# envoy/ksql

Hardware: AMD Instinct MI355X
Metric: records/sec, windowed GROUP BY (COUNT(*) TUMBLING 5 s GROUP BY card_number HAVING > 3) (higher is better)
Workload: dtype int64

## Files before the change

### ksql_amd/csrc/khip_agg_c1.hip

```cpp
#include <algorithm>
#include <cstdio>
#include <type_traits>
#include <vector>

#include "khip_part.hpp"

namespace khip {

constexpr int C1_TILE = 65536;
constexpr int C1_NT = 512;
constexpr int C1_CH = 8192;
template <class T>
__device__ __forceinline__ T c1_ld(const T* p) {
  return *p;
}
constexpr int C1_SEGMAX = 512;
constexpr int C1_SEGB = 7;
constexpr int C1_SEGOF = 512;
constexpr uint32_t C1_SENT = 0x80000000u;

__device__ __forceinline__ int bits_of(uint64_t v) { return v ? 64 - __clzll((long long)v) : 0; }

__device__ __forceinline__ int64_t ci_ld(const int64_t* ci, int k) {
  const uint64_t v = (uint64_t)__hip_atomic_load(&ci[k], __ATOMIC_RELAXED, __HIP_MEMORY_SCOPE_AGENT);
// ... 761 lines not shown
      for (int u = 0; u < AU; u++) any |= (uint32_t)sb[u] <= li[u];
      if (!__ballot(any)) break;
      for (int u = 0; u < AU; u++) {
        const bool on = (uint32_t)sb[u] <= li[u];
        lo[u] += on ? 1 : 0;
        ba[u] = on ? (uint32_t)(sb[u] >> 32) : ba[u];
        sb[u] = sg2[lo[u] + 1];
      }
    }
#pragma unroll
    for (int u = 0; u < AU; u++) at[u] = ba[u] + li[u];
  } else {
    uint32_t lo[AU], hi[AU];
#pragma unroll
    for (int u = 0; u < AU; u++) {
      lo[u] = 0u;
      hi[u] = (uint32_t)nseg;
    }
    for (int span = nseg; span > 1; span = (span + 1) >> 1) {
      uint32_t pm[AU];
#pragma unroll
      for (int u = 0; u < AU; u++) pm[u] = (uint32_t)sg2[(lo[u] + hi[u]) >> 1];
#pragma unroll
      for (int u = 0; u < AU; u++) {
        const uint32_t mid = (lo[u] + hi[u]) >> 1;
        const bool up = pm[u] <= li[u];
        lo[u] = up ? mid : lo[u];
        hi[u] = up ? hi[u] : mid;
      }
    }
#pragma unroll
    for (int u = 0; u < AU; u++) at[u] = (uint32_t)(sg2[lo[u]] >> 32) + li[u];
  }
}

template <int NT, int AU, class ID, bool WIDE>
__global__ __launch_bounds__(NT, 4) void k_c1_merge(
    C1Q q, const uint32_t* __restrict__ work, int64_t nwork, const int64_t* __restrict__ bb,
    const int* __restrict__ cstart, const uint16_t* __restrict__ seg, const uint64_t* __restrict__ srec, int first,
    uint64_t* __restrict__ buf0, uint64_t* __restrict__ buf1, const uint8_t* __restrict__ sel,
    const int64_t* __restrict__ cnt, unsigned long long* __restrict__ newcnt, uint8_t* __restrict__ fail,
    unsigned long long* __restrict__ need, int64_t close0, uint64_t* __restrict__ closed,
    unsigned long long* __restrict__ closed_n, unsigned long long closed_cap, const int64_t* __restrict__ ci,
    unsigned long long* __restrict__ hnew,
    unsigned long long* __restrict__ hclosed, uint32_t* __restrict__ prn, const uint32_t* __restrict__ srecT,
    unsigned long long* __restrict__ dbg) {
  if (ci_ld(ci, CI_GATE) == 0) return;
  if ((ci_ld(ci, CI_WIDE) != 0) != WIDE) return;
  if (!WIDE && (ci_ld(ci, CI_ID32) != 0) != (sizeof(ID) == 4)) return;
  static_assert(!WIDE || sizeof(ID) == 8, "wide records use 64-bit identities");
  constexpr int NW = NT / 64;
  constexpr ID EMPTY = (ID)~(ID)0;
  const int log2H = q.log2H;
  const int H = 1 << log2H;
  const int lane = threadIdx.x & 63, wave = threadIdx.x >> 6;
  extern __shared__ __attribute__((aligned(16))) char smem[];
  KLDS ID* ids = (KLDS ID*)(KLDS char*)smem;
  KLDS uint32_t* rt = (KLDS uint32_t*)((KLDS char*)smem + (size_t)(H + 64) * sizeof(ID));
  KLDS uint32_t* ct = rt + (H + 64);
  KLDS uint16_t* list = (KLDS uint16_t*)(ct + (H + 64));
  KLDS uint64_t* sg2 = (KLDS uint64_t*)((KLDS char*)list + (((size_t)H * 2 + 15) & ~(size_t)15));
  KLDS int64_t* lbb = (KLDS int64_t*)(sg2 + C1_SEGMAX + 4);
  KLDS int32_t* lcs = (KLDS int32_t*)(lbb + (1 << (q.log2P - q.fbits)) + 1);
  KLDS uint16_t* segof = (KLDS uint16_t*)(lcs + (1 << (q.log2P - q.fbits)) + 2);
  __shared__ int lovf, nnew;
  __shared__ int wsum[NW], csum[NW];
  __shared__ unsigned long long lbase, cbase;
  const int F = 1 << q.fbits;
  const int64_t wbase = ci_ld(ci, CI_WBASE), whi = ci_ld(ci, CI_WHI), T0 = ci_ld(ci, CI_T0), tmin = ci_ld(ci, CI_TMIN);
  const int wbits = (int)ci_ld(ci, CI_WBITS);
  const int64_t kmin = ci_ld(ci, CI_KMINC);
  const uint64_t krange = (uint64_t)ci_ld(ci, CI_KRANGE);
  const int32_t tmin32 = (int32_t)(tmin - T0);
  const int64_t wstart = wbase * q.adv;
  const bool r32 = ci_ld(ci, CI_TMAX) - wstart < ((int64_t)1 << 32);
  const uint32_t tsh32 = (uint32_t)(T0 - wstart);
  const bool evict = close0 != INT64_MIN;
  C1M_T0;
  const uint32_t dummy = (uint32_t)H + (uint32_t)lane;
  for (int i = threadIdx.x; i < H + 64; i += NT) {
    ids[i] = EMPTY;
    rt[i] = 0u;
    ct[i] = 0u;
  }
  if (threadIdx.x == 0) {
    lovf = 0;
    nnew = 0;
  }
  auto row_id = [&](const uint64_t* row, ID* id, uint32_t* h) -> bool {
    const int64_t wi = (int64_t)fast_udiv((uint64_t)row[1], q.fd) - wbase;
    if constexpr (WIDE) {
      if (wi < 0 || wi > whi) {
        *h = (uint32_t)(key_hash((int64_t)row[0]) >> 32) ^ (uint32_t)row[1];
        return false;
      }
      *id = (ID)((key_hash((int64_t)row[0]) << q.log2P) | (uint64_t)wi);
      *h = c1_hash<ID>(*id);
      return true;
    }
    const uint64_t krel = (uint64_t)((int64_t)row[0] - kmin);
    if (krel > krange || wi < 0 || wi > whi) {
      *h = (uint32_t)(key_hash((int64_t)row[0]) >> 32) ^ (uint32_t)row[1];
      return false;
    }
    if constexpr (sizeof(ID) == 4) *id = (ID)(((uint32_t)krel << wbits) | (uint32_t)wi);
    else *id = (ID)((krel << 32) | (uint64_t)wi);
    *h = c1_hash<ID>(*id);
    return true;
  };
  struct Pre {
    uint32_t p;
    int sbits, sub;
    int64_t nrow;
    uint32_t selw;
    uint32_t s0, s1;
  };
  auto bucket = [&](uint32_t p, int& cs, int64_t& bb0) -> int {
    const int b = (int)(p >> q.fbits);
    cs = lcs[b];
    bb0 = lbb[b];
    const int nseg = lcs[b + 1] - cs;
    return nseg < 0 || nseg > C1_SEGMAX ? 0 : nseg;
  };
  struct It {
    uint32_t p;
    int sbits, sub, nseg, segb;
    uint32_t rn;
    uint32_t bb0;
    int64_t nrow;
    bool isel;
  };
  auto fetch = [&](int64_t w, Pre& r) {
    uint32_t p;
    int sbits = 0, sub = 0;
    if (work) {
      const uint32_t x = work[w];
      p = x & 0xFFFFu;
      sbits = (x >> 16) & 0xF;
      sub = (int)(x >> 20);
    } else {
      p = (uint32_t)w;
    }
    p = __builtin_amdgcn_readfirstlane(p);
    const int f = (int)(p & (uint32_t)(F - 1));
    int cs;
    int64_t bb0;
    const int nseg = bucket(p, cs, bb0);
    r.p = p;
    r.sbits = sbits;
    r.sub = sub;
    r.nrow = cnt[p];
    r.selw = ((const uint32_t*)sel)[p >> 2];
    const int k0 = threadIdx.x * 2;
    r.s0 = r.s1 = 0u;
    if (k0 < nseg) {
      const uint16_t* sg = seg + (int64_t)(cs + k0) * (F + 1) + f;
      r.s0 = (uint32_t)sg[0] | (uint32_t)sg[1] << 16;
    }
    if (k0 + 1 < nseg) {
      const uint16_t* sg = seg + (int64_t)(cs + k0 + 1) * (F + 1) + f;
      r.s1 = (uint32_t)sg[0] | (uint32_t)sg[1] << 16;
    }
  };
  auto prep = [&](const Pre& r, It& it) {
    int cs;
    int64_t bb0;
    const int nseg = bucket(r.p, cs, bb0);
    it.p = r.p;
    it.sbits = r.sbits;
    it.sub = r.sub;
    it.nrow = r.nrow;
    it.isel = ((r.selw >> (8 * (r.p & 3))) & 0xFFu) != 0;
    const int k0 = threadIdx.x * 2;
    const uint32_t s00 = r.s0 & 0xFFFFu, s10 = r.s1 & 0xFFFFu;
    const int len0 = k0 < nseg ? (int)(r.s0 >> 16) - (int)s00 : 0;
    const int len1 = k0 + 1 < nseg ? (int)(r.s1 >> 16) - (int)s10 : 0;
    const uint32_t base0 = (uint32_t)(k0 * C1_CH) + s00;
    const uint32_t base1 = (uint32_t)((k0 + 1) * C1_CH) + s10;
    const int s = len0 + len1;
    int incl = s;
    for (int off = 1; off < 64; off <<= 1) {
      const int y = __shfl_up(incl, off, 64);
      if (lane >= off) incl += y;
    }
    if (lane == 63) wsum[wave] = incl;
    lds_barrier();
    int before = 0;
    int tot = 0;
    for (int k = 0; k < NW; k++) {
      before += k < wave ? wsum[k] : 0;
      tot += wsum[k];
    }
    const int ex = before + incl - s;
    const int segb = tot <= (C1_SEGOF << 5) ? 5 : (tot <= (C1_SEGOF << 6) ? 6 : C1_SEGB);
    const int bm = (1 << segb) - 1;
    if (k0 < nseg) sg2[k0] = (uint32_t)ex | (uint64_t)(base0 - (uint32_t)ex) << 32;
    if (k0 + 1 < nseg) sg2[k0 + 1] = (uint32_t)(ex + len0) | (uint64_t)(base1 - (uint32_t)(ex + len0)) << 32;
    for (int bj = (ex + bm) >> segb, be = (ex + len0 + bm) >> segb; bj < be && bj < C1_SEGOF; bj++)
      segof[bj] = (uint16_t)k0;
    for (int bj = (ex + len0 + bm) >> segb, be = (ex + s + bm) >> segb; bj < be && bj < C1_SEGOF; bj++)
      segof[bj] = (uint16_t)(k0 + 1);
    if (k0 < nseg && k0 + 2 >= nseg) sg2[nseg] = (uint32_t)(ex + s);
    if (nseg == 0 && threadIdx.x == 0) sg2[0] = 0u;
    lds_barrier();
    it.rn = __builtin_amdgcn_readfirstlane((uint32_t)sg2[nseg]);
    it.segb = __builtin_amdgcn_readfirstlane(segb);
    it.nseg = __builtin_amdgcn_readfirstlane(nseg);
    it.bb0 = __builtin_amdgcn_readfirstlane((uint32_t)bb0);
  };
  uint64_t ra[AU], rb[AU];
  uint32_t ta[AU], tb[AU];
  auto load = [&](uint64_t (&x)[AU], uint32_t (&tx)[AU], uint32_t l0, const It& t) {
    uint32_t at[AU];
    c1_seg_lookup<AU, NT>(sg2, segof, l0, t.rn, t.nseg, t.segb, at);
    const char* sb = (const char*)(srec + t.bb0);
#pragma unroll
    for (int u = 0; u < AU; u++) x[u] = c1_ld((const uint64_t*)(sb + (uint64_t)(uint32_t)(at[u] << 3)));
    if constexpr (WIDE) {
      const char* sbT = (const char*)(srecT + t.bb0);
#pragma unroll
      for (int u = 0; u < AU; u++) tx[u] = c1_ld((const uint32_t*)(sbT + (uint64_t)(uint32_t)(at[u] << 2)));
    }
  };
  auto load01 = [&](const It& x) {
    if (x.rn > 0) load(ra, ta, 0u, x);
    if (x.rn > (uint32_t)(AU * NT)) load(rb, tb, (uint32_t)(AU * NT), x);
  };
  for (int k = threadIdx.x; k <= (1 << (q.log2P - q.fbits)); k += NT) {
    lcs[k] = cstart[k];
    lbb[k] = bb[k];
  }
  lds_barrier();
  Pre pr{};
  It nx{};
  if (blockIdx.x < nwork) {
    fetch(blockIdx.x, pr);
    prep(pr, nx);
    load01(nx);
  }
  for (int64_t w = blockIdx.x; w < nwork; w += gridDim.x) {
    const It it = nx;
    const uint32_t p = it.p;
    const int sbits = it.sbits, sub = it.sub;
    const uint32_t rn = it.rn;
    const int64_t nrow = it.nrow;
    const bool isel = it.isel;
    const int64_t wn = w + gridDim.x;
    if (wn < nwork) fetch(wn, pr);
    if (first && threadIdx.x == 0) prn[p] = rn;
    if (rn == 0 && first) {
      if (wn < nwork) {
        prep(pr, nx);
        load01(nx);
      }
      continue;
    }
    const uint64_t* src = (isel ? buf1 : buf0) + (uint64_t)p * q.cmax * q.sw;
    auto evict_failed = [&]() {
      if (!first || !evict || nrow == 0) return;
      auto mine_closed = [&](const uint64_t* row) -> bool {
        if ((int64_t)row[1] + q.size > close0) return false;
        if (!sbits) return true;
        ID id;
        uint32_t h;
        row_id(row, &id, &h);
        return (int)c1_sub(h, sbits) == sub;
      };
      int n_cl = 0;
      for (int64_t r = threadIdx.x; r < nrow; r += NT) n_cl += mine_closed(src + r * q.sw) ? 1 : 0;
      const int wave_cl = (int)wave_sum(n_cl);
      if (lane == 0) csum[wave] = wave_cl;
      lds_barrier();
      int cl_before = 0, cl_total = 0;
      for (int k = 0; k < NW; k++) {
        if (k < wave) cl_before += csum[k];
        cl_total += csum[k];
      }
      if (threadIdx.x == 0)
        cbase = c1_reserve_closed(closed_n, (unsigned long long)cl_total, closed_cap, &fail[p], need);
      lds_barrier();
      const unsigned long long cb = cbase;
      if (cl_total == 0 || cb == C1_NOSLOT) return;
      uint64_t ccur = cb + (uint64_t)cl_before;
      const uint64_t lt = (1ULL << lane) - 1;
      int nhc = 0;
      for (int64_t r0 = wave * 64; r0 < nrow; r0 += NT) {
        const int64_t r = r0 + lane;
        const uint64_t* row = src + (r < nrow ? r : 0) * q.sw;
        const bool cl = r < nrow && mine_closed(row);
        const uint64_t bc = __ballot(cl);
        if (cl) {
          uint64_t* cd = closed + (ccur + __popcll(bc & lt)) * q.sw;
          for (int k = 0; k < q.sw; k++) cd[k] = row[k];
          nhc += q.hv_active && c1q_having(q, row[3]) ? 1 : 0;
        }
        ccur += __popcll(bc);
      }
      if (q.hv_active) {
        nhc = (int)wave_sum(nhc);
        if (lane == 0 && nhc) atomicAdd(hclosed, (unsigned long long)nhc);
      }
    };
    C1M_T(0);
    auto apply = [&](const uint64_t (&xr)[AU], const uint32_t (&txr)[AU], uint32_t l0, auto R32, auto&& prefetch) -> bool {
      ID id[AU];
      uint32_t e[AU], tr[AU];
      bool pend[AU], claimed[AU];
#pragma unroll
      for (int u = 0; u < AU; u++) {
        const uint32_t li = l0 + threadIdx.x + (uint32_t)(u * NT);
        const uint64_t v = xr[u];
        const int32_t t32 = WIDE ? (int32_t)txr[u] : (int32_t)(uint32_t)v;
        const uint64_t krel = v >> 32;
        uint64_t wi;
        if constexpr (decltype(R32)::value) wi = fast_udiv32((uint32_t)t32 + tsh32, q.fd32);
        else wi = fast_udiv((uint64_t)(T0 + (int64_t)t32), q.fd) - (uint64_t)wbase;
        ID x;
        if constexpr (WIDE) x = (ID)((v << q.log2P) | wi);
        else if constexpr (sizeof(ID) == 4) x = (ID)(((uint32_t)krel << wbits) | (uint32_t)wi);
        else x = (ID)((krel << 32) | wi);
        const uint32_t h = c1_hash<ID>(x);
        bool act = li < rn;
        if (sbits) act = act && (int)c1_sub(h, sbits) == sub;
        id[u] = act ? x : EMPTY;
        e[u] = act ? h >> (32 - log2H) : dummy;
        tr[u] = (uint32_t)(t32 - tmin32) + 1u;
      }
      ID old[AU];
#pragma unroll
      for (int u = 0; u < AU; u++) {
        old[u] = EMPTY;
        __hip_atomic_compare_exchange_strong(&ids[e[u]], &old[u], id[u], __ATOMIC_RELAXED, __ATOMIC_RELAXED,
                                             __HIP_MEMORY_SCOPE_WORKGROUP);
      }
      const int fullv = *(volatile KLDS int*)&lovf;
      prefetch();
      const int full = __builtin_amdgcn_readfirstlane(fullv);
#pragma unroll
      for (int u = 0; u < AU; u++) {
        claimed[u] = id[u] != EMPTY && old[u] == EMPTY;
        pend[u] = old[u] != EMPTY && old[u] != id[u];
      }
      for (int probes = 1;; probes++) {
        bool anyp = false;
#pragma unroll
        for (int u = 0; u < AU; u++) anyp |= pend[u];
        if (!__ballot(anyp)) break;
        if (probes >= H) {
          lovf = 1;
#pragma unroll
          for (int u = 0; u < AU; u++)
            if (pend[u]) id[u] = EMPTY;
          break;
        }
#pragma unroll
        for (int u = 0; u < AU; u++) {
          if (!pend[u]) continue;
          e[u] = (e[u] + 1) & (uint32_t)(H - 1);
          ID o2 = EMPTY;
          __hip_atomic_compare_exchange_strong(&ids[e[u]], &o2, id[u], __ATOMIC_RELAXED, __ATOMIC_RELAXED,
                                               __HIP_MEMORY_SCOPE_WORKGROUP);
          claimed[u] = o2 == EMPTY;
          pend[u] = o2 != EMPTY && o2 != id[u];
        }
      }
      int nnow;
      {
        bool cl[AU];
#pragma unroll
        for (int u = 0; u < AU; u++) cl[u] = claimed[u] && id[u] != EMPTY;
        nnow = mg_list_append_n<AU>(cl, e, list, &nnew);
      }
#pragma unroll
      for (int u = 0; u < AU; u++) {
        if (id[u] == EMPTY) continue;
        __hip_atomic_fetch_max(&rt[e[u]], tr[u], WG_RLX);
        __hip_atomic_fetch_add(&ct[e[u]], 1u, WG_RLX);
      }
      return !full && nnow <= q.hmax;
    };
    constexpr uint32_t CR = (uint32_t)(AU * NT);
    const uint32_t nch = (rn + CR - 1u) / CR;
    if (rn > 0) {
      for (uint32_t c = 0; c < nch; c += 2) {
        auto pa = [&] { if (c + 2 < nch) load(ra, ta, (c + 2) * CR, it); };
        const bool ga = r32 ? apply(ra, ta, c * CR, std::true_type{}, pa) : apply(ra, ta, c * CR, std::false_type{}, pa);
        if (!ga || c + 1 >= nch) break;
        auto pb = [&] { if (c + 3 < nch) load(rb, tb, (c + 3) * CR, it); };
        const bool gb = r32 ? apply(rb, tb, (c + 1) * CR, std::true_type{}, pb)
                            : apply(rb, tb, (c + 1) * CR, std::false_type{}, pb);
        if (!gb) break;
      }
    }
    lds_barrier();
    if (wn < nwork) {
      prep(pr, nx);
      load01(nx);
    }
    C1M_T(1);
    const int nl = nnew < H ? nnew : H;
    if (lovf || nnew > q.hmax) {
      if (threadIdx.x == 0) fail[p] |= 1;
      for (int i = threadIdx.x; i < nl; i += NT) {
        const uint32_t e = list[i];
        ids[e] = EMPTY;
        rt[e] = 0u;
        ct[e] = 0u;
      }
      evict_failed();
      lds_barrier();
      if (threadIdx.x == 0) {
        lovf = 0;
        nnew = 0;
      }
      lds_barrier();
      continue;
    }
    int n_mine = 0, n_cl = 0;
    for (int64_t r = threadIdx.x; r < nrow; r += NT) {
      const uint64_t* row = src + r * q.sw;
      ID id;
      uint32_t h;
      const bool has = row_id(row, &id, &h);
      if (sbits && (int)c1_sub(h, sbits) != sub) continue;
      if (evict && (int64_t)row[1] + q.size <= close0) {
        n_cl += first ? 1 : 0;
        continue;
      }
      if (has) {
        const int e = c1_find_id<ID>(ids, id, h >> (32 - log2H), H);
        if (e >= 0) rt[e] |= RT_MATCHED;
      }
      n_mine++;
    }
    if (nrow > 0) lds_barrier();
    const int per = ((nl + NW - 1) / NW + 63) & ~63;
    const int lb0 = wave * per, lb1 = lb0 + per < nl ? lb0 + per : nl;
    int nnw = 0;
    for (int k = lb0; k < lb1; k += 64) {
      const int i = k + lane;
      const uint32_t e = i < lb1 ? list[i] : dummy;
      const bool isnew = i < lb1 && !(rt[e] & RT_MATCHED);
      nnw += (int)__popcll(__ballot(isnew));
    }
    const int wave_rows = (int)wave_sum(n_mine) + nnw;
    const int wave_cl = (int)wave_sum(n_cl);
    if (lane == 0) {
      wsum[wave] = wave_rows;
      csum[wave] = wave_cl;
    }
    lds_barrier();
    int wave_before = 0, total = 0, cl_before = 0, cl_total = 0;
    for (int k = 0; k < NW; k++) {
      if (k < wave) wave_before += wsum[k], cl_before += csum[k];
      total += wsum[k];
      cl_total += csum[k];
    }
    if (threadIdx.x == 0) {
      if (work) lbase = total ? atomicAdd(&newcnt[p], (unsigned long long)total) : 0ULL;
      else {
        lbase = 0;
        newcnt[p] = (unsigned long long)total;
      }
      cbase = (int64_t)(lbase + total) <= q.cmax
                  ? c1_reserve_closed(closed_n, (unsigned long long)cl_total, closed_cap, &fail[p], need)
                  : 0ULL;
    }
    lds_barrier();
    if ((int64_t)(lbase + total) > q.cmax) {
      if (threadIdx.x == 0) {
        fail[p] |= 2;
        atomicMax(need, (unsigned long long)(lbase + total));
      }
      for (int i = threadIdx.x; i < nl; i += NT) {
        const uint32_t e = list[i];
        ids[e] = EMPTY;
        rt[e] = 0u;
        ct[e] = 0u;
      }
      evict_failed();
      lds_barrier();
      if (threadIdx.x == 0) nnew = 0;
      lds_barrier();
      continue;
    }
    C1M_T(3);
    uint64_t* dst0 = (isel ? buf0 : buf1) + (uint64_t)p * q.cmax * q.sw;
    uint64_t cur = lbase + (uint64_t)wave_before;
    uint64_t ccur = cbase + (uint64_t)cl_before;
    const bool cmove = first && cbase != C1_NOSLOT;
    const uint64_t lt = (1ULL << lane) - 1;
    int nh = 0, nhc = 0;
    for (int64_t r0 = wave * 64; r0 < nrow; r0 += NT) {
      const int64_t r = r0 + lane;
      const uint64_t* row = src + (r < nrow ? r : 0) * q.sw;
      bool live = r < nrow, cl = false;
      int e = -1;
      if (live) {
        ID id;
        uint32_t h;
        const bool has = row_id(row, &id, &h);
        if (sbits) live = (int)c1_sub(h, sbits) == sub;
        cl = live && evict && (int64_t)row[1] + q.size <= close0;
        live = live && !cl;
        if (live && has) e = c1_find_id<ID>(ids, id, h >> (32 - log2H), H);
      }
      const uint64_t bc = __ballot(cl);
      if (cl && cmove) {
        uint64_t* cd = closed + (ccur + __popcll(bc & lt)) * q.sw;
        for (int k = 0; k < q.sw; k++) cd[k] = row[k];
        nhc += q.hv_active && c1q_having(q, row[3]) ? 1 : 0;
      }
      ccur += __popcll(bc);
      const uint64_t bl = __ballot(live);
      if (live) {
        const uint64_t ri = cur + __popcll(bl & lt);
        uint64_t* dst = dst0 + ri * q.sw;
        uint64_t w2 = row[2], c = row[3];
        if (e >= 0) {
          const int64_t t = tmin + (int64_t)(rt[e] & ~RT_MATCHED) - 1;
          w2 = t > (int64_t)w2 ? (uint64_t)t : w2;
          c += ct[e];
        }
        *(longlong2*)dst = make_longlong2((int64_t)row[0], (int64_t)row[1]);
        *(longlong2*)(dst + 2) = make_longlong2((int64_t)w2, (int64_t)c);
        const bool now = !q.hv_active || c1q_having(q, c);
        nh += q.hv_active && now ? 1 : 0;
        if (q.chg)
          q.chg[(uint64_t)p * q.cmax + ri] =
              e >= 0 ? (uint8_t)(CHG_TOUCHED | (!q.hv_active || c1q_having(q, row[3]) ? CHG_OLD : 0) | (now ? CHG_NEW : 0))
                     : (uint8_t)0;
      }
      cur += __popcll(bl);
    }
    if (nrow > 0) lds_barrier();
    const uint32_t wmask = wbits ? (1u << wbits) - 1u : 0u;
    for (int k = lb0; k < lb1; k += 64) {
      const int i = k + lane;
      const uint32_t e = i < lb1 ? list[i] : dummy;
      const uint32_t rv = rt[e];
      const bool used = i < lb1;
      const bool isnew = used && !(rv & RT_MATCHED);
      const uint64_t bl = __ballot(isnew);
      if (isnew) {
        const uint64_t ri = cur + __popcll(bl & lt);
        uint64_t* dst = dst0 + ri * q.sw;
        const ID id = ids[e];
        int64_t key, wi;
        if constexpr (WIDE) {
          wi = (int64_t)((uint64_t)id & (((uint64_t)1 << q.log2P) - 1));
          key = key_of_hash(((uint64_t)p << (64 - q.log2P)) | ((uint64_t)id >> q.log2P));
        } else if constexpr (sizeof(ID) == 4) {
          key = kmin + (int64_t)((uint32_t)id >> wbits);
          wi = (int64_t)((uint32_t)id & wmask);
        } else {
          key = kmin + (int64_t)((uint64_t)id >> 32);
          wi = (int64_t)((uint64_t)id & 0xFFFFFFFFull);
        }
        const uint32_t c = ct[e];
        *(longlong2*)dst = make_longlong2(key, (wbase + wi) * q.adv);
        *(longlong2*)(dst + 2) = make_longlong2(tmin + (int64_t)rv - 1, (int64_t)c);
        const bool now = !q.hv_active || c1q_having(q, c);
        nh += q.hv_active && now ? 1 : 0;
        if (q.chg) q.chg[(uint64_t)p * q.cmax + ri] = (uint8_t)(CHG_TOUCHED | (now ? CHG_NEW : 0));
      }
      if (used) {
        ids[e] = EMPTY;
        rt[e] = 0u;
        ct[e] = 0u;
      }
      cur += __popcll(bl);
    }
    if (q.hv_active) {
      nh = (int)wave_sum(nh);
      nhc = (int)wave_sum(nhc);
      if (lane == 0 && nh) atomicAdd(&hnew[p], (unsigned long long)nh);
      if (lane == 0 && nhc) atomicAdd(hclosed, (unsigned long long)nhc);
    }
    lds_barrier();
    C1M_T(4);
    if (threadIdx.x == 0) nnew = 0;
    lds_barrier();
  }
}

constexpr int C1V_CH = 4096;
constexpr int C1V_MAXW = 8;

typedef uint64_t c1v_u2 __attribute__((ext_vector_type(2)));
__device__ __forceinline__ ulonglong2 ld_nt2(const ulonglong2* p) {
  const c1v_u2 v = c1_ld((const c1v_u2*)p);
  return make_ulonglong2(v.x, v.y);
}

struct C1VCol {
  const void* data;
  const uint8_t* valid;
  int32_t type;
};


template <int U, int NT, bool ST, bool ROWS>
__global__ __launch_bounds__(NT) __attribute__((amdgpu_waves_per_eu(4))) void k_c1v_scatter(
    const int64_t* __restrict__ keys, const int64_t* __restrict__ ts, const uint8_t* __restrict__ kv,
    const uint8_t* __restrict__ rv, C1VCol vc, RowsIn ri, int64_t n, int64_t nT, int log2B, uint16_t* __restrict__ rloc,
    uint16_t* __restrict__ roff, uint32_t* __restrict__ ttot, ulonglong2* __restrict__ srec, int64_t* __restrict__ tilestat,
    int64_t* __restrict__ tpart, int64_t* __restrict__ ci, const int64_t* __restrict__ st_at, int64_t size, int64_t adv,
    FastDiv fd, int hop, int64_t grace, const int64_t* __restrict__ stream_time, int64_t kb_in, int has_kb) {
  extern __shared__ __attribute__((aligned(16))) char smem[];
  __shared__ int wsum[NT / 64];
  __shared__ unsigned long long lc[5];
  __shared__ int lt[2][2];
  __shared__ int lfail, lkfail;
  __shared__ uint32_t lkr[2];
  constexpr int S = U * NT;
  constexpr int SPT = C1_TILE / S;
  const int B = 1 << log2B;
  const int64_t t = tile_of(blockIdx.x, nT);
  uint32_t* cnt = (uint32_t*)smem;
  uint32_t* sbase = cnt + B;
  ulonglong2* sp = (ulonglong2*)(smem + (size_t)B * 8);
  uint32_t* lrc = (uint32_t*)(smem + run_stage_lds(B, S, 16, false));
  uint16_t* lro = (uint16_t*)(lrc + SPT * B);
  for (int b = threadIdx.x; b < B; b += NT) cnt[b] = 0u;
  if (threadIdx.x < 5) lc[threadIdx.x] = 0;
  if (threadIdx.x < 2) {
    lt[threadIdx.x][0] = INT32_MIN;
    lt[threadIdx.x][1] = INT32_MAX;
  }
  if (threadIdx.x == 0) {
    lfail = lkfail = 0;
    lkr[0] = 0xFFFFFFFFu;
    lkr[1] = 0u;
  }
  int64_t T0, kb;
  if constexpr (ROWS) run_bases((const int64_t*)ri.rows, (const int64_t*)ri.rows + 1, n, stream_time, kb_in, has_kb, 31, ci, &T0, &kb);
  else run_bases(keys, ts, n, stream_time, kb_in, has_kb, 31, ci, &T0, &kb);
  const int shift = log2B == 0 ? 64 : 64 - log2B;
  const uint32_t bmask = (uint32_t)(B - 1);
  const int64_t base = t * C1_TILE;
  const int64_t end = base + C1_TILE < n ? base + C1_TILE : n;
  int c_acc = 0, c_nk = 0, c_nr = 0, c_bt = 0, c_app = 0;
  uint32_t kor = 0u;
  int64_t x[U], k[U], v[U];
  uint32_t vm[ROWS ? U : 1];
  int64_t rst[ROWS && ST ? U : 1];
  auto load_step = [&](int64_t i0) {
#pragma unroll
    for (int u = 0; u < U; u++) {
      int64_t i = i0 + (int64_t)u * NT;
      i = i < end ? i : end - 1;
      if constexpr (ROWS) {
        const uint64_t* r = ri.rows + i * (int64_t)ri.rw;
        if (ri.rw == 4 && ri.vword == 2) {
          const ulonglong2 a = ((const ulonglong2*)r)[0], b = ((const ulonglong2*)r)[1];
          k[u] = (int64_t)a.x;
          x[u] = (int64_t)a.y;
          v[u] = (int64_t)b.x;
          vm[u] = (uint32_t)b.y;
        } else {
          k[u] = (int64_t)r[0];
          x[u] = (int64_t)r[1];
          v[u] = (int64_t)r[ri.vword];
          vm[u] = (uint32_t)r[ri.rw - 1];
        }
        if constexpr (ST) rst[u] = (int64_t)r[ri.rw - 2];
      } else {
        x[u] = ts[i];
        k[u] = keys[i];
        v[u] = vc.type == KHIP_TYPE_INT32 ? (int64_t)((const int32_t*)vc.data)[i] : ((const int64_t*)vc.data)[i];
      }
    }
  };
  int64_t t_rmax = -1, t_min = INT64_MAX, t_bound = INT64_MAX;
  bool t_ok = true;
  auto publish = [&](int64_t, int st) {
    const int mx = lt[st & 1][0], mn = lt[st & 1][1];
    if (mx != INT32_MIN) {
      const int64_t smx = T0 + mx, smn = T0 + mn;
      t_rmax = smx > t_rmax ? smx : t_rmax;
      t_min = smn < t_min ? smn : t_min;
      const int64_t fw = first_window_start_fd(smn, size, adv, fd) + size;
      const int64_t b = grace > ((int64_t)1 << 61) ? INT64_MAX : fw + grace - 1;
      t_bound = b < t_bound ? b : t_bound;
      t_ok = t_ok && t_rmax <= b;
    }
    lt[st & 1][0] = INT32_MIN;
    lt[st & 1][1] = INT32_MAX;
  };
  lds_barrier();
  int64_t s0 = base;
  int st_last = -1;
  if (s0 < end) load_step(s0 + threadIdx.x);
  for (int st = 0; s0 < end; s0 += S, st++) {
    st_last = st;
    const int64_t i0 = s0 + threadIdx.x;
    bool ok[U];
    uint32_t bin[U];
    ulonglong2 rec[U];
    int tmx = INT32_MIN, tmn = INT32_MAX;
#pragma unroll
    for (int u = 0; u < U; u++) {
      const int64_t i = i0 + (int64_t)u * NT;
      ok[u] = i < end;
      const int64_t ii = ok[u] ? i : base;
      const bool kok = ROWS || bit_get(kv, ii), rok = ROWS || bit_get(rv, ii);
      const bool vok = ROWS ? ((vm[ROWS ? u : 0] >> ri.vbit) & 1u) != 0 : bit_get(vc.valid, ii);
      const bool valid = ok[u] && kok && rok && x[u] >= 0;
      c_nk += ok[u] && !kok;
      c_nr += ok[u] && kok && !rok;
      c_bt += ok[u] && kok && rok && x[u] < 0;
      c_acc += valid;
      const int64_t d = x[u] - T0;
      if (valid && (d <= (int64_t)INT32_MIN || d > (int64_t)INT32_MAX)) {
        lfail = 1;
#ifdef KHIP_TUNING
        if (ci[CI_N - 1] == 1 && (threadIdx.x & 63) == 0) printf("[c1 scatter] t %ld i %ld x %ld T0 %ld\n", (long)t, (long)i, (long)x[u], (long)T0);
#endif
      }
      if constexpr (ST) {
        const int64_t ds = (ROWS ? rst[ROWS ? u : 0] : st_at[ii]) - T0;
        if (valid && (ds <= (int64_t)INT32_MIN || ds > (int64_t)INT32_MAX)) lfail = 1;
        tmx = valid && (int)ds > tmx ? (int)ds : tmx;
      } else {
        tmx = valid && (int)d > tmx ? (int)d : tmx;
      }
      tmn = valid && (int)d < tmn ? (int)d : tmn;
      if (hop && valid) {
        const int64_t lo = x[u] - size + adv;
        c_app += (int)((int64_t)fast_udiv((uint64_t)x[u], fd) - (int64_t)fast_udiv((uint64_t)(lo > 0 ? lo : 0), fd) + 1);
      }
      bin[u] = stage_bin(key_hash(k[u]), shift, bmask);
      const uint64_t kd = (uint64_t)k[u] - (uint64_t)kb;
      kor |= ok[u] ? (uint32_t)(kd >> 31) : 0u;
      const uint64_t w0 = ((kd & 0x7FFFFFFFull) << 32) | (uint64_t)(valid ? (uint32_t)d : C1_SENT);
      rec[u] = make_ulonglong2(w0 | (vok ? (1ULL << 63) : 0ULL), (uint64_t)v[u]);
    }
    if (s0 + S < end) load_step(i0 + S);
    uint32_t t32u[U];
    const uint32_t tot = stage_step_runs<U, NT, ulonglong2, false>(rec, t32u, bin, ok, B, cnt, sbase, wsum, sp, nullptr,
                                                                   srec, nullptr, t * SPT + st, lrc + st * B,
                                                                   lro + st * B);
    step_krange<NT, ulonglong2>(sp, tot, 0x7FFFFFFFu, lkr);
    for (int off = 32; off > 0; off >>= 1) {
      const int a = __shfl_xor(tmx, off, 64), b = __shfl_xor(tmn, off, 64);
      tmx = a > tmx ? a : tmx;
      tmn = b < tmn ? b : tmn;
    }
    if ((threadIdx.x & 63) == 0 && tmx != INT32_MIN) {
      atomicMax(&lt[st & 1][0], tmx);
      atomicMin(&lt[st & 1][1], tmn);
    }
    if (threadIdx.x == 0 && st > 0) publish(s0 - S, st - 1);
  }
  flush_run_counts<SPT, NT>(lrc, lro, B, st_last, t, nT, rloc, roff, ttot);
  if (kor) lkfail = 1;
  __syncthreads();
  if (threadIdx.x == 0 && s0 > base) publish(s0 - S, st_last);
  if (threadIdx.x == 0) run_krange(lkr, lkfail, kb, ci);
  c_acc = wave_sum(c_acc);
  c_nk = wave_sum(c_nk);
  c_nr = wave_sum(c_nr);
  c_bt = wave_sum(c_bt);
  c_app = wave_sum(c_app);
  if ((threadIdx.x & 63) == 0) {
    if (c_acc) atomicAdd(&lc[0], (unsigned long long)c_acc);
    if (c_nk) atomicAdd(&lc[1], (unsigned long long)c_nk);
    if (c_nr) atomicAdd(&lc[2], (unsigned long long)c_nr);
    if (c_bt) atomicAdd(&lc[3], (unsigned long long)c_bt);
    if (c_app) atomicAdd(&lc[4], (unsigned long long)c_app);
  }
  __syncthreads();
  if (threadIdx.x == 0) {
    int64_t* tp = tpart + t * T_NPART;
    tp[T_ACCEPTED] = (int64_t)lc[0];
    tp[T_NULL_KEY] = (int64_t)lc[1];
    tp[T_NULL_ROW] = (int64_t)lc[2];
    tp[T_BAD_TS] = (int64_t)lc[3];
    tp[T_APPLIED] = hop ? (int64_t)lc[4] : (int64_t)lc[0];
    tp[T_LATE] = 0;
    if (lfail) atomicOr((unsigned long long*)&ci[CI_TFAIL], 1ULL);
    int64_t* ts4 = tilestat + t * 4;
    ts4[0] = t_rmax;
    ts4[1] = t_min;
    ts4[2] = t_bound;
    ts4[3] = t_ok ? 1 : 0;
  }
}

template <int U, int NT>
__global__ __launch_bounds__(NT) __attribute__((amdgpu_waves_per_eu(4))) void k_c1v_refine(
    const ulonglong2* __restrict__ srcA, const int64_t* __restrict__ bb, const int* __restrict__ cstart, int log2B,
    int log2P, int fbits, ulonglong2* __restrict__ srec, uint16_t* __restrict__ seg, const int64_t* __restrict__ ci,
    const uint32_t* __restrict__ tbase, const uint16_t* __restrict__ rloc, const uint16_t* __restrict__ roff,
    int64_t nT, int sh, int64_t S, const uint32_t* __restrict__ cinfo) {
  if (ci_ld(ci, CI_GATE) == 0) return;
  const int w = blockIdx.x;
  if (w >= (int)ci_ld(ci, CI_NCHUNK)) return;
  extern __shared__ __attribute__((aligned(16))) char smem[];
  __shared__ int lb, lnv;
  __shared__ int wsum[NT / 64];
  constexpr int CH = U * NT;
  static_assert(CH == C1V_CH, "refine chunk");
  const int F = 1 << fbits, B = 1 << log2B;
  uint32_t* cnt = (uint32_t*)smem;
  uint32_t* sbase = cnt + F;
  ulonglong2* stage = (ulonglong2*)(smem + (((size_t)F * 8 + 15) & ~(size_t)15));
  for (int f = threadIdx.x; f < F; f += NT) cnt[f] = 0u;
  if (threadIdx.x == 0) lb = -1;
  __syncthreads();
  for (int b = threadIdx.x; b < B; b += NT)
    if (cstart[b] <= w && w < cstart[b + 1]) lb = b;
  __syncthreads();
  const int b = lb;
  if (b < 0) return;
  const int64_t lo = bb[b] + (int64_t)(w - cstart[b]) * CH;
  const int64_t bend = bb[b + 1];
  const int len = (int)(bend - lo < CH ? bend - lo : CH);
  const int64_t kmin = ci_ld(ci, CI_KMINC);
  const uint64_t kshift = (uint64_t)ci_ld(ci, CI_KSHIFT) << 32;
  const int shift = 64 - log2P;
  const int64_t nSt = nT << sh;
  chunk_map(tbase + (int64_t)b * (nT + 1), rloc + (int64_t)b * nSt, roff + (int64_t)b * nSt, nSt, sh, cinfo, w, S,
            lo - bb[b], len, (uint32_t*)stage);
  ulonglong2 r[U];
  uint32_t f[U], rank[U];
#pragma unroll
  for (int u = 0; u < U; u++) {
    const int j = threadIdx.x + u * NT;
    const uint32_t src = ((const uint32_t*)stage)[j < len ? j : len - 1];
    r[u] = ld_nt2(srcA + src);
    r[u].x -= kshift;
  }
#pragma unroll
  for (int u = 0; u < U; u++) {
    const int j = threadIdx.x + u * NT;
    const bool v = j < len && (uint32_t)r[u].x != C1_SENT;
    f[u] = (uint32_t)(key_hash(kmin + (int64_t)((r[u].x >> 32) & 0x7FFFFFFFull)) >> shift) & (uint32_t)(F - 1);
    rank[u] = v ? atomicAdd(&cnt[f[u]], 1u) : 0xFFFFFFFFu;
  }
  __syncthreads();
  {
    const int t = threadIdx.x, lane = t & 63, wave = t >> 6;
    const uint32_t c = t < F ? cnt[t] : 0u;
    uint32_t incl = c;
    for (int off = 1; off < 64; off <<= 1) {
      const uint32_t y = __shfl_up(incl, off, 64);
      if (lane >= off) incl += y;
    }
    if (lane == 63) wsum[wave] = (int)incl;
    __syncthreads();
    uint32_t before = 0, tot = 0;
#pragma unroll
    for (int k = 0; k < NT / 64; k++) {
      before += k < wave ? (uint32_t)wsum[k] : 0u;
      tot += (uint32_t)wsum[k];
    }
    if (t < F) {
      sbase[t] = before + incl - c;
      seg[(int64_t)w * (F + 1) + t] = (uint16_t)(before + incl - c);
    }
    if (t == 0) {
      seg[(int64_t)w * (F + 1) + F] = (uint16_t)tot;
      lnv = (int)tot;
    }
  }
  __syncthreads();
  const int nv = lnv;
#pragma unroll
  for (int u = 0; u < U; u++)
    if (rank[u] != 0xFFFFFFFFu) stage[sbase[f[u]] + rank[u]] = r[u];
  __syncthreads();
  for (int j = threadIdx.x; j < nv; j += NT) srec[lo + j] = stage[j];
}

struct C1VQ {
  int32_t log2P, fbits, log2H, sw, hmax, f64, fan;
  int32_t off_sum, off_min, off_max, off_rt, off_star, off_cnt, off_list, off_spre;
  int32_t word_op[C1V_MAXW];
  int64_t size, adv, cmax;
  FastDiv fd;
  FastDiv32 fd32;
  uint64_t init[C1V_MAXW];
  HavingDev having;
  uint8_t* chg;
// ... 1208 lines not shown
```

Measured before the change: 57.99 billion.

## Trim tail-chunk work and barriers in C1 windowed aggregation loop

Specializes the final partial chunk of the hash-insert loop to process only 1 or 2 unrolled slots instead of the full AU, which avoids wasted CAS work on inactive lanes. It also snapshots nnew/lovf into registers right after the barrier and resets them early, removing the extra lds_barrier pairs at the end of each iteration and on the failure paths. When there are no existing rows, it skips the per-wave prefix-sum and closed reservation and uses the list size directly, saving a barrier. The added complexity raises the risk of race or ordering bugs around the shared nnew/lovf resets.

```diff
diff --git a/ksql_amd/csrc/khip_agg_c1.hip b/ksql_amd/csrc/khip_agg_c1.hip
--- a/ksql_amd/csrc/khip_agg_c1.hip
+++ b/ksql_amd/csrc/khip_agg_c1.hip
@@ -1087,12 +1087,14 @@
       }
     };
     C1M_T(0);
-    auto apply = [&](const uint64_t (&xr)[AU], const uint32_t (&txr)[AU], uint32_t l0, auto R32, auto&& prefetch) -> bool {
-      ID id[AU];
-      uint32_t e[AU], tr[AU];
-      bool pend[AU], claimed[AU];
-#pragma unroll
-      for (int u = 0; u < AU; u++) {
+    auto apply = [&](const uint64_t (&xr)[AU], const uint32_t (&txr)[AU], uint32_t l0, auto R32, auto NUc,
+                     auto&& prefetch) -> bool {
+      constexpr int NU = decltype(NUc)::value;
+      ID id[NU];
+      uint32_t e[NU], tr[NU];
+      bool pend[NU], claimed[NU];
+#pragma unroll
+      for (int u = 0; u < NU; u++) {
         const uint32_t li = l0 + threadIdx.x + (uint32_t)(u * NT);
         const uint64_t v = xr[u];
         const int32_t t32 = WIDE ? (int32_t)txr[u] : (int32_t)(uint32_t)v;
@@ -1111,9 +1113,9 @@
         e[u] = act ? h >> (32 - log2H) : dummy;
         tr[u] = (uint32_t)(t32 - tmin32) + 1u;
       }
-      ID old[AU];
-#pragma unroll
-      for (int u = 0; u < AU; u++) {
+      ID old[NU];
+#pragma unroll
+      for (int u = 0; u < NU; u++) {
         old[u] = EMPTY;
         __hip_atomic_compare_exchange_strong(&ids[e[u]], &old[u], id[u], __ATOMIC_RELAXED, __ATOMIC_RELAXED,
                                              __HIP_MEMORY_SCOPE_WORKGROUP);
@@ -1122,24 +1124,24 @@
       prefetch();
       const int full = __builtin_amdgcn_readfirstlane(fullv);
 #pragma unroll
-      for (int u = 0; u < AU; u++) {
+      for (int u = 0; u < NU; u++) {
         claimed[u] = id[u] != EMPTY && old[u] == EMPTY;
         pend[u] = old[u] != EMPTY && old[u] != id[u];
       }
       for (int probes = 1;; probes++) {
         bool anyp = false;
 #pragma unroll
-        for (int u = 0; u < AU; u++) anyp |= pend[u];
+        for (int u = 0; u < NU; u++) anyp |= pend[u];
         if (!__ballot(anyp)) break;
         if (probes >= H) {
           lovf = 1;
 #pragma unroll
-          for (int u = 0; u < AU; u++)
+          for (int u = 0; u < NU; u++)
             if (pend[u]) id[u] = EMPTY;
           break;
         }
 #pragma unroll
-        for (int u = 0; u < AU; u++) {
+        for (int u = 0; u < NU; u++) {
           if (!pend[u]) continue;
           e[u] = (e[u] + 1) & (uint32_t)(H - 1);
           ID o2 = EMPTY;
@@ -1151,13 +1153,13 @@
       }
       int nnow;
       {
-        bool cl[AU];
-#pragma unroll
-        for (int u = 0; u < AU; u++) cl[u] = claimed[u] && id[u] != EMPTY;
-        nnow = mg_list_append_n<AU>(cl, e, list, &nnew);
-      }
-#pragma unroll
-      for (int u = 0; u < AU; u++) {
+        bool cl[NU];
+#pragma unroll
+        for (int u = 0; u < NU; u++) cl[u] = claimed[u] && id[u] != EMPTY;
+        nnow = mg_list_append_n<NU>(cl, e, list, &nnew);
+      }
+#pragma unroll
+      for (int u = 0; u < NU; u++) {
         if (id[u] == EMPTY) continue;
         __hip_atomic_fetch_max(&rt[e[u]], tr[u], WG_RLX);
         __hip_atomic_fetch_add(&ct[e[u]], 1u, WG_RLX);
@@ -1166,25 +1168,59 @@
     };
     constexpr uint32_t CR = (uint32_t)(AU * NT);
     const uint32_t nch = (rn + CR - 1u) / CR;
+    constexpr int TAILNU = AU - 1 < 2 ? AU - 1 : 2;
+    const uint32_t tail_r = rn - (nch - 1u) * CR;
+    const uint32_t tnu =
+        rn > 0 && tail_r <= (uint32_t)(TAILNU * NT) ? (tail_r + (uint32_t)(NT - 1)) / (uint32_t)NT : (uint32_t)AU;
+    const uint32_t nfc = tnu < (uint32_t)AU ? nch - 1u : nch;
+    using FullNU = std::integral_constant<int, AU>;
     if (rn > 0) {
-      for (uint32_t c = 0; c < nch; c += 2) {
+      bool go = true;
+      for (uint32_t c = 0; c < nfc; c += 2) {
         auto pa = [&] { if (c + 2 < nch) load(ra, ta, (c + 2) * CR, it); };
-        const bool ga = r32 ? apply(ra, ta, c * CR, std::true_type{}, pa) : apply(ra, ta, c * CR, std::false_type{}, pa);
-        if (!ga || c + 1 >= nch) break;
+        const bool ga = r32 ? apply(ra, ta, c * CR, std::true_type{}, FullNU{}, pa)
+                            : apply(ra, ta, c * CR, std::false_type{}, FullNU{}, pa);
+        if (!ga) go = false;
+        if (!ga || c + 1 >= nfc) break;
         auto pb = [&] { if (c + 3 < nch) load(rb, tb, (c + 3) * CR, it); };
-        const bool gb = r32 ? apply(rb, tb, (c + 1) * CR, std::true_type{}, pb)
-                            : apply(rb, tb, (c + 1) * CR, std::false_type{}, pb);
-        if (!gb) break;
+        const bool gb = r32 ? apply(rb, tb, (c + 1) * CR, std::true_type{}, FullNU{}, pb)
+                            : apply(rb, tb, (c + 1) * CR, std::false_type{}, FullNU{}, pb);
+        if (!gb) {
+          go = false;
+          break;
+        }
+      }
+      if (go && nfc < nch) {
+        auto tail = [&](const uint64_t (&xr)[AU], const uint32_t (&txr)[AU], auto NUc) {
+          auto none = [] {};
+          if (r32) apply(xr, txr, nfc * CR, std::true_type{}, NUc, none);
+          else apply(xr, txr, nfc * CR, std::false_type{}, NUc, none);
+        };
+        using N1 = std::integral_constant<int, 1>;
+        using N2 = std::integral_constant<int, TAILNU>;
+        if (nfc & 1u) {
+          if (tnu == 1u) tail(rb, tb, N1{});
+          else tail(rb, tb, N2{});
+        } else {
+          if (tnu == 1u) tail(ra, ta, N1{});
+          else tail(ra, ta, N2{});
+        }
       }
     }
     lds_barrier();
+    const int nnew_r = __builtin_amdgcn_readfirstlane(nnew);
+    const int lovf_r = __builtin_amdgcn_readfirstlane(lovf);
     if (wn < nwork) {
       prep(pr, nx);
+      if (threadIdx.x == 0) {
+        lovf = 0;
+        nnew = 0;
+      }
       load01(nx);
     }
     C1M_T(1);
-    const int nl = nnew < H ? nnew : H;
-    if (lovf || nnew > q.hmax) {
+    const int nl = nnew_r < H ? nnew_r : H;
+    if (lovf_r || nnew_r > q.hmax) {
       if (threadIdx.x == 0) fail[p] |= 1;
       for (int i = threadIdx.x; i < nl; i += NT) {
         const uint32_t e = list[i];
@@ -1193,11 +1229,6 @@
         ct[e] = 0u;
       }
       evict_failed();
-      lds_barrier();
-      if (threadIdx.x == 0) {
-        lovf = 0;
-        nnew = 0;
-      }
       lds_barrier();
       continue;
     }
@@ -1221,41 +1252,58 @@
     if (nrow > 0) lds_barrier();
     const int per = ((nl + NW - 1) / NW + 63) & ~63;
     const int lb0 = wave * per, lb1 = lb0 + per < nl ? lb0 + per : nl;
-    int nnw = 0;
-    for (int k = lb0; k < lb1; k += 64) {
-      const int i = k + lane;
-      const uint32_t e = i < lb1 ? list[i] : dummy;
-      const bool isnew = i < lb1 && !(rt[e] & RT_MATCHED);
-      nnw += (int)__popcll(__ballot(isnew));
-    }
-    const int wave_rows = (int)wave_sum(n_mine) + nnw;
-    const int wave_cl = (int)wave_sum(n_cl);
-    if (lane == 0) {
-      wsum[wave] = wave_rows;
-      csum[wave] = wave_cl;
-    }
-    lds_barrier();
     int wave_before = 0, total = 0, cl_before = 0, cl_total = 0;
-    for (int k = 0; k < NW; k++) {
-      if (k < wave) wave_before += wsum[k], cl_before += csum[k];
-      total += wsum[k];
-      cl_total += csum[k];
-    }
-    if (threadIdx.x == 0) {
-      if (work) lbase = total ? atomicAdd(&newcnt[p], (unsigned long long)total) : 0ULL;
-      else {
-        lbase = 0;
-        newcnt[p] = (unsigned long long)total;
-      }
-      cbase = (int64_t)(lbase + total) <= q.cmax
-                  ? c1_reserve_closed(closed_n, (unsigned long long)cl_total, closed_cap, &fail[p], need)
-                  : 0ULL;
-    }
-    lds_barrier();
-    if ((int64_t)(lbase + total) > q.cmax) {
+    unsigned long long lb, cb;
+    if (nrow == 0) {
+      total = nl;
+      wave_before = lb0 < nl ? lb0 : nl;
+      cb = 0ULL;
+      if (work) {
+        if (threadIdx.x == 0) lbase = total ? atomicAdd(&newcnt[p], (unsigned long long)total) : 0ULL;
+        lds_barrier();
+        lb = lbase;
+      } else {
+        lb = 0ULL;
+        if (threadIdx.x == 0) newcnt[p] = (unsigned long long)total;
+      }
+    } else {
+      int nnw = 0;
+      for (int k = lb0; k < lb1; k += 64) {
+        const int i = k + lane;
+        const uint32_t e = i < lb1 ? list[i] : dummy;
+        const bool isnew = i < lb1 && !(rt[e] & RT_MATCHED);
+        nnw += (int)__popcll(__ballot(isnew));
+      }
+      const int wave_rows = (int)wave_sum(n_mine) + nnw;
+      const int wave_cl = (int)wave_sum(n_cl);
+      if (lane == 0) {
+        wsum[wave] = wave_rows;
+        csum[wave] = wave_cl;
+      }
+      lds_barrier();
+      for (int k = 0; k < NW; k++) {
+        if (k < wave) wave_before += wsum[k], cl_before += csum[k];
+        total += wsum[k];
+        cl_total += csum[k];
+      }
+      if (threadIdx.x == 0) {
+        if (work) lbase = total ? atomicAdd(&newcnt[p], (unsigned long long)total) : 0ULL;
+        else {
+          lbase = 0;
+          newcnt[p] = (unsigned long long)total;
+        }
+        cbase = (int64_t)(lbase + total) <= q.cmax
+                    ? c1_reserve_closed(closed_n, (unsigned long long)cl_total, closed_cap, &fail[p], need)
+                    : 0ULL;
+      }
+      lds_barrier();
+      lb = lbase;
+      cb = cbase;
+    }
+    if ((int64_t)(lb + total) > q.cmax) {
       if (threadIdx.x == 0) {
         fail[p] |= 2;
-        atomicMax(need, (unsigned long long)(lbase + total));
+        atomicMax(need, (unsigned long long)(lb + total));
       }
       for (int i = threadIdx.x; i < nl; i += NT) {
         const uint32_t e = list[i];
@@ -1265,15 +1313,13 @@
       }
       evict_failed();
       lds_barrier();
-      if (threadIdx.x == 0) nnew = 0;
-      lds_barrier();
       continue;
     }
     C1M_T(3);
     uint64_t* dst0 = (isel ? buf0 : buf1) + (uint64_t)p * q.cmax * q.sw;
-    uint64_t cur = lbase + (uint64_t)wave_before;
-    uint64_t ccur = cbase + (uint64_t)cl_before;
-    const bool cmove = first && cbase != C1_NOSLOT;
+    uint64_t cur = lb + (uint64_t)wave_before;
+    uint64_t ccur = cb + (uint64_t)cl_before;
+    const bool cmove = first && cb != C1_NOSLOT;
     const uint64_t lt = (1ULL << lane) - 1;
     int nh = 0, nhc = 0;
     for (int64_t r0 = wave * 64; r0 < nrow; r0 += NT) {
@@ -1364,8 +1410,6 @@
     }
     lds_barrier();
     C1M_T(4);
-    if (threadIdx.x == 0) nnew = 0;
-    lds_barrier();
   }
 }
 
```

Result: faster. 60.05 billion (median of 6 runs) (+3.5%).
